# rgal/gym-2048

Hardware: AMD Instinct MI355X
Metric: env-steps/sec at batch=2^20 per MI355X (higher is better)
Workload: dtype u8

## Files before the change

### gym-2048_amd/csrc/g2048_device.h

```cpp
#pragma once

#include <stdint.h>

#if defined(G2048_HOST_CHECK)
#define G2048_DEV static inline
static inline uint32_t g2048_perm(uint32_t hi, uint32_t lo, uint32_t sel)
{
    uint64_t src = ((uint64_t)hi << 32) | lo;
    uint32_t out = 0;
    for (int k = 0; k < 4; ++k) {
        uint32_t s = (sel >> (8 * k)) & 0xff;
        uint32_t byte = s < 8 ? (uint32_t)((src >> (8 * s)) & 0xff) : (s == 12 ? 0u : 0xffu);
        out |= byte << (8 * k);
    }
    return out;
}
static inline uint32_t g2048_mulhi(uint32_t a, uint32_t b) { return (uint32_t)(((uint64_t)a * b) >> 32); }
static inline uint32_t g2048_popc(uint32_t x) { return (uint32_t)__builtin_popcount(x); }
static inline uint32_t g2048_clz(uint32_t x) { return (uint32_t)__builtin_clz(x); }
static inline uint32_t g2048_funnel_shr(uint32_t hi, uint32_t lo, uint32_t k)
{
    return (uint32_t)(((((uint64_t)hi) << 32) | lo) >> (k & 31u));
}
static inline uint32_t g2048_ctz(uint32_t x) { return (uint32_t)__builtin_ctz(x); }
static inline float g2048_rcp(float x) { return 1.0f / x; }
static inline uint32_t g2048_opaque(uint32_t x) { return x; }
static inline uint32_t g2048_bfi(uint32_t m, uint32_t a, uint32_t b) { return (m & a) | (~m & b); }
static inline bool g2048_any(bool x) { return x; }
static inline uint32_t g2048_xor3(uint32_t a, uint32_t b, uint32_t c) { return a ^ b ^ c; }
template <int K> static inline uint32_t g2048_pow2_byte(uint32_t x, uint32_t) { return 1u << ((x >> (8 * K)) & 31u); }
#else
#include <hip/hip_runtime.h>
#define G2048_DEV __device__ __forceinline__
G2048_DEV uint32_t g2048_perm(uint32_t hi, uint32_t lo, uint32_t sel) { return __builtin_amdgcn_perm(hi, lo, sel); }
G2048_DEV uint32_t g2048_mulhi(uint32_t a, uint32_t b) { return __umulhi(a, b); }
G2048_DEV uint32_t g2048_popc(uint32_t x) { return (uint32_t)__popc(x); }
G2048_DEV uint32_t g2048_clz(uint32_t x) { return (uint32_t)__builtin_clz(x); }
G2048_DEV uint32_t g2048_funnel_shr(uint32_t hi, uint32_t lo, uint32_t k) { return __builtin_amdgcn_alignbit(hi, lo, k); }
G2048_DEV uint32_t g2048_ctz(uint32_t x) { return (uint32_t)__builtin_ctz(x); }
G2048_DEV float g2048_rcp(float x) { return __builtin_amdgcn_rcpf(x); }
G2048_DEV uint32_t g2048_opaque(uint32_t x)
{
    asm volatile("" : "+v"(x));
    return x;
}
G2048_DEV uint32_t g2048_bfi(uint32_t m, uint32_t a, uint32_t b) { return __builtin_amdgcn_bitop3_b32(m, a, b, 0xCA); }
G2048_DEV uint32_t g2048_xor3(uint32_t a, uint32_t b, uint32_t c) { return __builtin_amdgcn_bitop3_b32(a, b, c, 0x96); }
template <int K> G2048_DEV uint32_t g2048_pow2_byte(uint32_t x, uint32_t one)
{
    uint32_t r;
    if constexpr (K == 0)
        asm("v_lshlrev_b32_sdwa %0, %1, %2 dst_sel:DWORD dst_unused:UNUSED_PAD src0_sel:BYTE_0 src1_sel:DWORD" : "=v"(r) : "v"(x), "v"(one));
    else if constexpr (K == 1)
        asm("v_lshlrev_b32_sdwa %0, %1, %2 dst_sel:DWORD dst_unused:UNUSED_PAD src0_sel:BYTE_1 src1_sel:DWORD" : "=v"(r) : "v"(x), "v"(one));
    else if constexpr (K == 2)
        asm("v_lshlrev_b32_sdwa %0, %1, %2 dst_sel:DWORD dst_unused:UNUSED_PAD src0_sel:BYTE_2 src1_sel:DWORD" : "=v"(r) : "v"(x), "v"(one));
    else
        asm("v_lshlrev_b32_sdwa %0, %1, %2 dst_sel:DWORD dst_unused:UNUSED_PAD src0_sel:BYTE_3 src1_sel:DWORD" : "=v"(r) : "v"(x), "v"(one));
    return r;
}
G2048_DEV bool g2048_any(bool x) { return __builtin_amdgcn_ballot_w64(x) != 0ull; }
#endif

namespace g2048 {

struct Board {
    uint32_t r[4];
};

#if defined(G2048_HOST_CHECK)
struct uint4 {
    uint32_t x, y, z, w;
};
G2048_DEV Board load_board(const uint4 *boards, uint32_t i)
{
    Board b;
    __builtin_memcpy(b.r, boards + i, 16);
    return b;
}
#else
// ... 151 lines not shown
    bd.r[3] |= tile & h2;
    return n;
}

G2048_DEV uint32_t add_tile(Board &bd, uint32_t w, uint32_t enable = 0xffffffffu)
{
    bool is2;
    return add_tile(bd, w, enable, is2);
}

G2048_DEV bool fresh_is_four_16(uint32_t w1) { return (w1 << 4) > kTwoThreshold; }
G2048_DEV bool fresh_is_four_15(uint32_t w2) { return w2 * 15u > kTwoThreshold; }

G2048_DEV Board fresh_board(uint32_t w1, uint32_t w2)
{
    const uint32_t p1 = w1 >> 28;
    const uint32_t k2 = g2048_mulhi(w2, 15u);
    const uint32_t p2 = k2 + (k2 >= p1 ? 1u : 0u);
    const uint32_t e1 = fresh_is_four_16(w1) ? 2u : 1u;
    const uint32_t e2 = fresh_is_four_15(w2) ? 2u : 1u;
    const uint64_t x1 = (uint64_t)e1 << (8u * (p1 & 7u)), x2 = (uint64_t)e2 << (8u * (p2 & 7u));
    const uint32_t h1 = lanemask_bit0(p1 >> 3), h2 = lanemask_bit0(p2 >> 3);
    const uint32_t x1l = (uint32_t)x1, x1h = (uint32_t)(x1 >> 32), x2l = (uint32_t)x2, x2h = (uint32_t)(x2 >> 32);
    Board bd;
    bd.r[0] = (x1l & ~h1) | (x2l & ~h2);
    bd.r[1] = (x1h & ~h1) | (x2h & ~h2);
    bd.r[2] = (x1l & h1) | (x2l & h2);
    bd.r[3] = (x1h & h1) | (x2h & h2);
    return bd;
}

G2048_DEV bool has_equal_neighbours(const Board &bd)
{
    uint32_t f = 0;
#pragma unroll
    for (int i = 0; i < 4; ++i)
        f |= z80(bd.r[i] ^ (bd.r[i] >> 8)) & 0x00808080u;
#pragma unroll
    for (int i = 0; i < 3; ++i)
        f |= z80(bd.r[i] ^ bd.r[i + 1]);
    return f != 0;
}

G2048_DEV uint32_t max4(uint32_t x, uint32_t y)
{
    const uint32_t ge = mask7(((x | kHigh1) - y) & kHigh1);
    return bfi(ge, x, y);
}

G2048_DEV uint32_t highest(const Board &bd)
{
    uint32_t m = max4(max4(bd.r[0], bd.r[1]), max4(bd.r[2], bd.r[3]));
    m = max4(m, m >> 16);
    m = max4(m, m >> 8);
    return m & 0xffu;
}

G2048_DEV bool is_end(const Board &bd, uint32_t max_exp)
{
    bool end = false;
    if (count_empty(bd) == 0)
        end = !has_equal_neighbours(bd);
    if (max_exp != 0 && highest(bd) == max_exp)
        end = true;
    return end;
}

struct MoveSel {
    uint32_t sa, sb, ta, tc, va, vb;
};

#define G2048_MOVE_LUT_WORDS                                                                        \
    0x03020100u, 0x07060504u, 0x03020100u, 0x07060504u, 0x03020100u, 0x07060504u, 0u, 0u,      \
    0x05010703u, 0x04000602u, 0x05040100u, 0x07060302u, 0x00040206u, 0x01050307u, 0u, 0u,   \
// ... 1123 lines not shown
}

G2048_DEV uint32_t record_deficit(const Board &raw) { return gather12(raw.r[2]) | (gather12(raw.r[3]) << 12); }

G2048_DEV uint32_t record_score(const Board &raw)
{
    return (potential(record_cells(raw)) - record_deficit(raw)) & kScoreMask;
}

G2048_DEV Board make_record(const Board &cells, uint32_t score)
{
    const uint32_t d = (potential(cells) - score) & kScoreMask;
    return Board{{cells.r[0], cells.r[1], cells.r[2] | scatter12(d & 0xfffu), cells.r[3] | scatter12(d >> 12)}};
}

G2048_DEV void record_update(Board &raw, const Board &cells, uint32_t inc_spread)
{
    const uint64_t filled = (static_cast<uint64_t>(raw.r[3] | kCellBits) << 32) | (raw.r[2] | kCellBits);
    const uint64_t sum = filled + inc_spread;
    raw.r[0] = cells.r[0];
    raw.r[1] = cells.r[1];
    raw.r[2] = bfi(kSpareBits, static_cast<uint32_t>(sum), cells.r[2]);
    raw.r[3] = bfi(kSpareBits, static_cast<uint32_t>(sum >> 32), cells.r[3]);
}

G2048_DEV Board fresh_record(uint32_t w1, uint32_t w2)
{
    Board bd = fresh_board(w1, w2);
    const uint32_t fours = (fresh_is_four_16(w1) ? 1u : 0u) + (fresh_is_four_15(w2) ? 1u : 0u);
    bd.r[2] |= fours == 1u ? 0x80u : (fours == 2u ? 0x2000u : 0u);
    return bd;
}

template <class Tables>
G2048_DEV Board fresh_record_lut(uint32_t w1, uint32_t w2, const Tables &tb)
{
    const uint32_t p1 = w1 >> 28;
    const uint32_t k2 = g2048_mulhi(w2, 15u);
    const uint32_t p2 = k2 + (k2 >= p1 ? 1u : 0u);
    const uint32_t s1 = fresh_is_four_16(w1) ? 1u : 0u;
    const uint32_t s2 = fresh_is_four_15(w2) ? 1u : 0u;
    const Board a = tb.onehot_cell(p1), b = tb.onehot_cell(p2);
    const uint32_t fours = s1 + s2;
    Board bd;
    bd.r[0] = (a.r[0] << s1) | (b.r[0] << s2);
    bd.r[1] = (a.r[1] << s1) | (b.r[1] << s2);
    bd.r[2] = (a.r[2] << s1) | (b.r[2] << s2) | ((fours & 1u) << 7) | ((fours >> 1) << 13);
    bd.r[3] = (a.r[3] << s1) | (b.r[3] << s2);
    return bd;
}

G2048_DEV uint32_t onehot_cell_word(uint32_t p, uint32_t j) { return (p >> 2) == j ? 1u << (8u * (p & 3u)) : 0u; }

G2048_DEV uint32_t eq_flags(uint32_t cells, uint32_t splat) { return (kHigh1 - (cells ^ splat)) & kHigh1; }
G2048_DEV uint32_t eq_ones(uint32_t cells, uint32_t splat) { return ((kHigh1 - (cells ^ splat)) >> 7) & 0x01010101u; }

struct OneHot4F16 { uint32_t lo, hi; };
struct OneHot4F32 { uint32_t w[4]; };

G2048_DEV OneHot4F16 onehot4_f16(uint32_t cells, uint32_t splat)
{
    const uint32_t f = eq_flags(cells, splat);
    const uint32_t g = (f - (f >> 7)) & 0x3c3c3c3cu;
    return OneHot4F16{g2048_perm(g, g, 0x010c000cu), g2048_perm(g, g, 0x030c020cu)};
}

G2048_DEV OneHot4F32 onehot4_f32(uint32_t cells, uint32_t splat)
{
    const uint32_t f = eq_flags(cells, splat);
    const uint32_t g = (f - (f >> 7)) & 0x3f3f3f3fu;
    return OneHot4F32{{g2048_perm(g, f, 0x04000c0cu), g2048_perm(g, f, 0x05010c0cu), g2048_perm(g, f, 0x06020c0cu),
                       g2048_perm(g, f, 0x07030c0cu)}};
}

struct alignas(16) Cells16 { uint32_t r[4]; };
struct alignas(16) Chunk16 { uint32_t w[4]; };

template <int OBS>
G2048_DEV Chunk16 onehot_chunk(const Cells16 *recs, uint32_t s, uint32_t lane, uint32_t &board)
{
    if constexpr (OBS == 0) {
// ... 177 lines not shown
```

### gym-2048_amd/csrc/g2048_kernels.hip

```cpp
#include "g2048_kernels.h"

#include "g2048_device.h"
#include "g2048_pcg64.h"

#include <atomic>
#include <type_traits>


namespace g2048 {

constexpr int kBlock = 256;

typedef uint32_t u32x4 __attribute__((ext_vector_type(4)));

__device__ __forceinline__ Board load_board_nt(const uint4 *boards, uint32_t i)
{
    const u32x4 v = __builtin_nontemporal_load(reinterpret_cast<const u32x4 *>(boards) + i);
    return Board{{v.x, v.y, v.z, v.w}};
}

__device__ __forceinline__ void store_board_nt(uint4 *boards, uint32_t i, const Board &b)
{
    const u32x4 v = {b.r[0], b.r[1], b.r[2], b.r[3]};
    __builtin_nontemporal_store(v, reinterpret_cast<u32x4 *>(boards) + i);
}

__device__ __forceinline__ void store_chunk_nt(uint4 *out, uint64_t g, uint32_t a, uint32_t b, uint32_t c, uint32_t d)
{
    const u32x4 v = {a, b, c, d};
    __builtin_nontemporal_store(v, reinterpret_cast<u32x4 *>(out) + g);
}

__device__ __forceinline__ void store_board(uint4 *boards, uint32_t i, const Board &b)
{
    boards[i] = make_uint4(b.r[0], b.r[1], b.r[2], b.r[3]);
}

struct WaveTables {
    uint32_t move[32];
    uint32_t cell[64];
    uint32_t pad[32];
};

#define G2048_CELL_ENTRY(p) ((p) / 4 == 0 ? 1u << (8 * ((p) % 4)) : 0u), ((p) / 4 == 1 ? 1u << (8 * ((p) % 4)) : 0u), \
                            ((p) / 4 == 2 ? 1u << (8 * ((p) % 4)) : 0u), ((p) / 4 == 3 ? 1u << (8 * ((p) % 4)) : 0u)
__device__ const uint32_t kWaveTablesImage[128] __attribute__((aligned(16))) = {
    G2048_MOVE_LUT_WORDS,
    G2048_CELL_ENTRY(0), G2048_CELL_ENTRY(1), G2048_CELL_ENTRY(2), G2048_CELL_ENTRY(3),
    G2048_CELL_ENTRY(4), G2048_CELL_ENTRY(5), G2048_CELL_ENTRY(6), G2048_CELL_ENTRY(7),
    G2048_CELL_ENTRY(8), G2048_CELL_ENTRY(9), G2048_CELL_ENTRY(10), G2048_CELL_ENTRY(11),
    G2048_CELL_ENTRY(12), G2048_CELL_ENTRY(13), G2048_CELL_ENTRY(14), G2048_CELL_ENTRY(15),
};
#undef G2048_CELL_ENTRY

__device__ __forceinline__ uint2 use_after(uint2 x, uint32_t dep)
{
    unsigned long long both = (static_cast<unsigned long long>(x.y) << 32) | x.x;
    asm volatile("" : "+v"(both) : "v"(dep));
    return make_uint2(static_cast<uint32_t>(both), static_cast<uint32_t>(both >> 32));
}

struct LdsTables {
    const WaveTables *t;
    __device__ __forceinline__ MoveSel move_sel(uint32_t action) const
    {
        const uint4 a = *reinterpret_cast<const uint4 *>(t->move + action * 8u);
        const uint2 b = *reinterpret_cast<const uint2 *>(t->move + action * 8u + 4u);
        return MoveSel{a.x, a.y, a.z, a.w, b.x, b.y};
    }
    __device__ __forceinline__ Board onehot_cell(uint32_t p) const
    {
        const uint4 v = *reinterpret_cast<const uint4 *>(t->cell + p * 4u);
        return Board{{v.x, v.y, v.z, v.w}};
    }
};

__device__ __forceinline__ uint2 load_tables_piece()
{
    return reinterpret_cast<const uint2 *>(kWaveTablesImage)[threadIdx.x & 63u];
}

__device__ __forceinline__ LdsTables stage_tables(WaveTables *all, uint2 piece)
{
    reinterpret_cast<uint2 *>(all)[threadIdx.x] = piece;
    __builtin_amdgcn_fence(__ATOMIC_RELEASE, "wavefront");
    __builtin_amdgcn_fence(__ATOMIC_ACQUIRE, "wavefront");
    return LdsTables{all + (threadIdx.x >> 6)};
}

struct Lane { uint32_t i_raw, i; bool valid; };
template <uint32_t BLOCK, bool FULL> __device__ __forceinline__ Lane lane_of(uint32_t n)
{
    const uint32_t i_raw = blockIdx.x * BLOCK + threadIdx.x;
    const bool valid = FULL || i_raw < n;
    return Lane{i_raw, valid ? i_raw : n - 1u, valid};
}

template <int ACT> struct RawAction { typedef uint32_t type; };
template <> struct RawAction<1> { typedef uint8_t type; };
template <> struct RawAction<2> { typedef int32_t type; };
template <> struct RawAction<3> { typedef long long type; };
template <int ACT>
__device__ __forceinline__ typename RawAction<ACT>::type load_action_at(const void *__restrict__ actions, size_t idx)
{
    if constexpr (ACT == 0)
        return 0u;
    else
        return __builtin_nontemporal_load(static_cast<const typename RawAction<ACT>::type *>(actions) + idx);
}

template <class Raw> __device__ __forceinline__ uint32_t action_bits(Raw raw) { return static_cast<uint32_t>(raw) & 3u; }

__device__ __forceinline__ void report_bad_action(unsigned long long *action_err, bool bad, uint32_t raw_low, uint32_t global_index)
{
    const unsigned long long offenders = __builtin_amdgcn_ballot_w64(bad);
    if (offenders == 0ull)
        return;
// ... 1 lines not shown
        __hip_atomic_store(action_err, (1ull << 63) | (static_cast<unsigned long long>(raw_low & 0xffu) << 32) | global_index,
                           __ATOMIC_RELAXED, __HIP_MEMORY_SCOPE_SYSTEM);
}

struct BadAction {
    bool bad = false; uint32_t raw = 0;
    template <class Raw> __device__ __forceinline__ static bool outside(Raw v)
    {
        typedef typename std::make_unsigned<Raw>::type U;
        return static_cast<U>(v) > static_cast<U>(3);
    }
    template <class Raw> __device__ __forceinline__ uint32_t note_only(Raw v)
    {
        const auto w = static_cast<typename std::conditional<(sizeof(Raw) > 4), unsigned long long, uint32_t>::type>(v);
        bad = outside(w);
        raw = static_cast<uint32_t>(w);
        return action_bits(w);
    }
};

__device__ __forceinline__ unsigned long long record_episode_ends(const StepArgs &p, uint32_t i, bool fin, bool illegal,
                                                                  const Board &terminal, uint32_t &episodes, uint32_t &illegal_ends)
{
    const unsigned long long done = __builtin_amdgcn_ballot_w64(fin);
    if (done == 0ull)
        return 0ull;
    if (fin) {
        if (p.st.last_record)
            store_board(p.st.last_record, i, terminal);
        if (p.terminal_boards)
            store_board(p.terminal_boards, i, record_cells(terminal));
    }
    episodes += static_cast<uint32_t>(__popcll(done));
    illegal_ends += static_cast<uint32_t>(__popcll(__builtin_amdgcn_ballot_w64(fin && illegal)));
    return done;
}

__device__ __forceinline__ uint32_t wave_sum_lane63(uint32_t v)
{
    v += static_cast<uint32_t>(__builtin_amdgcn_update_dpp(0, static_cast<int>(v), 0x111, 0xf, 0xf, false));
    v += static_cast<uint32_t>(__builtin_amdgcn_update_dpp(0, static_cast<int>(v), 0x112, 0xf, 0xf, false));
    v += static_cast<uint32_t>(__builtin_amdgcn_update_dpp(0, static_cast<int>(v), 0x114, 0xf, 0xf, false));
    v += static_cast<uint32_t>(__builtin_amdgcn_update_dpp(0, static_cast<int>(v), 0x118, 0xf, 0xf, false));
    v += static_cast<uint32_t>(__builtin_amdgcn_update_dpp(0, static_cast<int>(v), 0x142, 0xa, 0xf, false));
    v += static_cast<uint32_t>(__builtin_amdgcn_update_dpp(0, static_cast<int>(v), 0x143, 0xc, 0xf, false));
    return v;
}

__device__ __forceinline__ unsigned long long wave_sum64_lane63(unsigned long long v)
{
    const uint32_t s0 = wave_sum_lane63(static_cast<uint32_t>(v) & 0x3fffffu);
    const uint32_t s1 = wave_sum_lane63(static_cast<uint32_t>(v >> 22) & 0x3fffffu);
    const uint32_t s2 = wave_sum_lane63(static_cast<uint32_t>(v >> 44));
    return static_cast<unsigned long long>(s0) + (static_cast<unsigned long long>(s1) << 22) +
           (static_cast<unsigned long long>(s2) << 44);
}

struct EpisodeCounters {
    uint32_t *slot;
    uint32_t ep_lo, ill_lo, gain_lo, pend_lo, ep_hi, ill_hi, gain_hi, pend_hi;
};

__device__ __forceinline__ uint32_t *slot_of(unsigned long long *ep_counters, uint32_t wave_id)
{
    return reinterpret_cast<uint32_t *>(ep_counters + kSlotWords * wave_id);
}

__device__ __forceinline__ EpisodeCounters load_episode_counters(const StepArgs &p, uint32_t i_raw)
{
    uint32_t *slot = slot_of(p.st.ep_counters, __builtin_amdgcn_readfirstlane(i_raw >> 6));
    const uint4 lo = *reinterpret_cast<const uint4 *>(slot), hi = *reinterpret_cast<const uint4 *>(slot + 4);
    return EpisodeCounters{slot, lo.x, lo.y, lo.z, lo.w, hi.x, hi.y, hi.z, hi.w};
}

__device__ __forceinline__ unsigned long long slot_get(const uint32_t *slot, uint32_t k)
{
    return static_cast<unsigned long long>(slot[k]) | (static_cast<unsigned long long>(slot[4u + k]) << 32);
}

__device__ __forceinline__ void slot_set(uint32_t *slot, uint32_t k, unsigned long long v)
{
    slot[k] = static_cast<uint32_t>(v);
    slot[4u + k] = static_cast<uint32_t>(v >> 32);
}

enum : uint32_t { kSlotEpisodes = 0, kSlotIllegal = 1, kSlotGain = 2, kSlotPending = 3 };

__device__ __forceinline__ void flush_episode_counts(const EpisodeCounters &c, uint32_t episodes, uint32_t illegal_ends,
                                                     unsigned long long gain_lane63, unsigned long long pending)
{
    if ((threadIdx.x & 63u) != 63u)
        return;
    const unsigned long long ep = (static_cast<unsigned long long>(c.ep_hi) << 32 | c.ep_lo) + episodes;
    const unsigned long long ill = (static_cast<unsigned long long>(c.ill_hi) << 32 | c.ill_lo) + illegal_ends;
    const unsigned long long gain = (static_cast<unsigned long long>(c.gain_hi) << 32 | c.gain_lo) + gain_lane63;
    typedef uint32_t u32x3 __attribute__((ext_vector_type(3)));
    const u32x3 lo = {static_cast<uint32_t>(ep), static_cast<uint32_t>(ill), static_cast<uint32_t>(gain)};
    *reinterpret_cast<u32x3 *>(c.slot) = lo;
    const uint32_t ep_hi = static_cast<uint32_t>(ep >> 32), ill_hi = static_cast<uint32_t>(ill >> 32),
                   gain_hi = static_cast<uint32_t>(gain >> 32);
    if (ep_hi != c.ep_hi || ill_hi != c.ill_hi || gain_hi != c.gain_hi) {
        const u32x3 hi = {ep_hi, ill_hi, gain_hi};
        *reinterpret_cast<u32x3 *>(c.slot + 4) = hi;
    }
    const uint32_t pend_lo = static_cast<uint32_t>(pending), pend_hi = static_cast<uint32_t>(pending >> 32);
    if (pend_lo != c.pend_lo || pend_hi != c.pend_hi) {
        c.slot[3] = pend_lo;
        c.slot[7] = pend_hi;
    }
}

__device__ __forceinline__ unsigned long long pending_after_step(unsigned long long done, uint32_t auto_reset)
{
    return done & (0ull - static_cast<unsigned long long>(auto_reset == 0u ? 1u : 0u));
}

__device__ __forceinline__ void adjust_slot(unsigned long long *ep_counters, uint32_t i_raw, int32_t delta, bool clear)
{
    const uint32_t total = wave_sum_lane63(static_cast<uint32_t>(delta));
    const unsigned long long cleared = __builtin_amdgcn_ballot_w64(clear);
    if ((threadIdx.x & 63u) == 63u) {
        uint32_t *slot = slot_of(ep_counters, i_raw >> 6);
        slot_set(slot, kSlotGain, slot_get(slot, kSlotGain) + static_cast<unsigned long long>(static_cast<long long>(static_cast<int32_t>(total))));
        slot_set(slot, kSlotPending, slot_get(slot, kSlotPending) & ~cleared);
    }
}

__device__ __forceinline__ bool is_pending(unsigned long long *ep_counters, uint32_t i_raw)
{
    const unsigned long long pending = slot_get(slot_of(ep_counters, __builtin_amdgcn_readfirstlane(i_raw >> 6)), kSlotPending);
    return ((pending >> (threadIdx.x & 63u)) & 1ull) != 0ull;
}

constexpr uint32_t kObsOccupancyPad = 58u * 1024u;

static_assert(sizeof(WaveTables) * (kBlock / 64) + sizeof(uint4) * kBlock + kObsOccupancyPad <= 64u * 1024u,
              "static LDS + occupancy pad exceed the 64 KiB workgroup limit");

template <auto Kernel>
static uint32_t obs_pad_for()
{
    static std::atomic<signed char> state[64] = {};
    int dev = 0;
    if (hipGetDevice(&dev) != hipSuccess || dev < 0 || dev >= 64)
        dev = 0;
    signed char known = state[dev].load(std::memory_order_acquire);
    if (known == 0) {
        const hipError_t err = hipFuncSetAttribute(reinterpret_cast<const void *>(Kernel), hipFuncAttributeMaxDynamicSharedMemorySize,
                                                   static_cast<int>(kObsOccupancyPad));
        if (err != hipSuccess)
            (void)hipGetLastError();
        known = err == hipSuccess ? 1 : -1;
        state[dev].store(known, std::memory_order_release);
    }
    return known > 0 ? kObsOccupancyPad : 0u;
}

template <int OBS, bool FULL>
__device__ __forceinline__ void emit_onehot_as(const Cells16 *recs, uint4 *out, uint32_t lane, uint32_t n_here)
{
    constexpr uint32_t kStores = 16u << OBS;
    constexpr uint32_t kUnroll = OBS == 2 ? 16u : kStores;
#pragma unroll kUnroll
    for (uint32_t s = 0; s < kStores; ++s) {
        uint32_t b;
        const Chunk16 c = onehot_chunk<OBS>(recs, s, lane, b);
        if (FULL || b < n_here)
            store_chunk_nt(out, s * 64u + lane, c.w[0], c.w[1], c.w[2], c.w[3]);
    }
}
// ... 80 lines not shown
step_args(uint4 *boards, const void *actions, unsigned long long *ep_counters, uint32_t board_offset, uint32_t seed_lo, uint32_t seed_hi,
          uint32_t t_lo, uint32_t t_hi, uint32_t n, float *reward, const StepTail &tail)
{
    StepArgs p{};
    p.st.boards = boards;
    p.st.last_record = tail.last_record;
    p.st.ep_counters = ep_counters;
    p.actions = actions;
    p.reward = reward;
    p.terminated = tail.terminated;
    p.illegal = STD ? nullptr : tail.illegal;
    p.highest = STD ? nullptr : tail.highest;
    p.terminal_boards = STD ? nullptr : tail.terminal_boards;
    p.n = n;
    p.board_offset = board_offset;
    p.seed_lo = seed_lo;
    p.seed_hi = seed_hi;
    p.t_lo = t_lo;
    p.t_hi = t_hi;
    p.illegal_reward = tail.illegal_reward;
    p.max_exp = STD ? 0u : tail.max_exp;
    p.auto_reset = tail.auto_reset;
    return p;
}

template <int ACT, bool FULL, bool STD, bool HAS_OBS>
__device__ __forceinline__ void step_body(WaveTables *s_tables, uint4 *s_recs, uint4 *boards, const void *actions,
                                          unsigned long long *ep_counters, uint32_t board_offset, uint32_t seed_lo, uint32_t seed_hi,
                                          uint32_t t_lo, uint32_t t_hi, uint32_t n, float *reward, const StepTail &tail)
{
    const StepArgs p = step_args<STD>(boards, actions, ep_counters, board_offset, seed_lo, seed_hi, t_lo, t_hi, n, reward, tail);
    const Lane ln = lane_of<kBlock, FULL>(p.n);
    Board rec = load_board_nt(p.st.boards, ln.i);
    const uint2 tables_piece = load_tables_piece();
    const EpisodeCounters counters = load_episode_counters(p, ln.i_raw);

    const Words w = philox4x32_10(p.t_lo, p.t_hi, p.board_offset + ln.i, 0u, p.seed_lo, p.seed_hi);
    BadAction bad;
    const uint32_t action = ACT == 0 ? w.w[3] >> 30 : bad.note_only(load_action_at<ACT>(p.actions, ln.i));
    const LdsTables tb = stage_tables(s_tables, use_after(tables_piece, w.w[0]));

    const StepOut o = play_record(rec, action, w, p.max_exp, tb);

    uint32_t episodes = 0, illegal_ends = 0;
    const unsigned long long done = record_episode_ends(p, ln.i, o.terminated && ln.valid, !o.legal, rec, episodes, illegal_ends);
    const uint32_t wave_gain = wave_sum_lane63(ln.valid ? o.gain : 0u);
    const unsigned long long pending = pending_after_step(done, p.auto_reset);
    uint32_t top = 0;
    if (p.highest)
        top = highest(record_cells(rec));
    if (o.terminated && p.auto_reset != 0)
        reset_record(rec, o, w, tb);

    if (ln.valid) {
        store_board_nt(p.st.boards, ln.i, rec);
        if (STD || p.reward)
            __builtin_nontemporal_store(o.legal ? static_cast<float>(o.gain) : p.illegal_reward, p.reward + ln.i);
        if (STD || p.terminated)
            __builtin_nontemporal_store(static_cast<uint8_t>(o.terminated ? 1 : 0), p.terminated + ln.i);
        if (p.illegal)
            __builtin_nontemporal_store(static_cast<uint8_t>(o.legal ? 0 : 1), p.illegal + ln.i);
        if (p.highest)
            __builtin_nontemporal_store(static_cast<uint8_t>(top), p.highest + ln.i);
        if (!STD && tail.boards_out)
            store_board(tail.boards_out, ln.i, record_cells(rec));
    }
    flush_episode_counts(counters, episodes, illegal_ends, wave_gain, pending);
    if constexpr (!STD && ACT != 0) {
        if (tail.action_err)
            report_bad_action(tail.action_err, bad.bad && ln.valid, bad.raw, p.board_offset + ln.i);
    }
    if constexpr (HAS_OBS)
        emit_onehot<FULL>(s_recs + (threadIdx.x & ~63u), rec, tail.obs, tail.obs_dtype, ln.i_raw & ~63u, n);
    if (!STD && tail.done_seq)
        signal_done(tail.done_seq, tail.done_value);
}

template <int ACT, bool FULL, bool STD, bool HAS_OBS>
// ... 13 lines not shown
        *t_ptr = value;
}

template <int ACT, bool FULL>
__global__ void __launch_bounds__(kBlock)
step_graph_kernel(uint4 *boards, const void *actions, unsigned long long *ep_counters, uint32_t board_offset, uint32_t seed_lo,
                  uint32_t seed_hi, const unsigned long long *t_ptr, uint32_t n, uint32_t j, float *reward, const StepTail tail)
{
    __shared__ WaveTables s_tables[kBlock / 64];
    const unsigned long long t = *t_ptr + j;
    step_body<ACT, FULL, true, false>(s_tables, nullptr, boards, actions, ep_counters, board_offset, seed_lo, seed_hi,
                                      static_cast<uint32_t>(t), static_cast<uint32_t>(t >> 32), n, reward, tail);
}

constexpr uint32_t kGainFold = 1024;
__global__ void __launch_bounds__(kBlock) rollout_random_kernel(const StepArgs p)
{
    __shared__ WaveTables s_tables[kBlock / 64];
    const Lane ln = lane_of<kBlock, false>(p.n);
    Board rec = load_board(p.st.boards, ln.i);
    const LdsTables tb = stage_tables(s_tables, load_tables_piece());
    const EpisodeCounters counters = load_episode_counters(p, ln.i_raw);
    uint64_t t = (static_cast<uint64_t>(p.t_hi) << 32) | p.t_lo;
    uint32_t episodes = 0, illegal_ends = 0;
    unsigned long long gained = 0;
    for (uint32_t j0 = 0; j0 < p.k_steps; j0 += kGainFold) {
        const uint32_t j1 = p.k_steps - j0 < kGainFold ? p.k_steps : j0 + kGainFold;
        uint32_t gained32 = 0;
        for (uint32_t j = j0; j < j1; ++j, ++t) {
            const Words w = philox4x32_10(static_cast<uint32_t>(t), static_cast<uint32_t>(t >> 32), p.board_offset + ln.i, 0u,
                                          p.seed_lo, p.seed_hi);
            const StepOut o = play_record(rec, w.w[3] >> 30, w, p.max_exp, tb);
            gained32 += o.gain;
            record_episode_ends(p, ln.i, o.terminated && ln.valid, !o.legal, rec, episodes, illegal_ends);
            if (o.terminated)
                reset_record(rec, o, w, tb);
        }
        gained += gained32;
    }
    if (ln.valid)
        store_board(p.st.boards, ln.i, rec);
    flush_episode_counts(counters, episodes, illegal_ends, wave_sum64_lane63(ln.valid ? gained : 0ull), 0ull);
}

constexpr uint32_t kPrefetch = 4;

template <int ACT>
__global__ void __launch_bounds__(kBlock) rollout_fused_kernel(const StepArgs p, uint64_t stride)
{
    __shared__ WaveTables s_tables[kBlock / 64];
    const Lane ln = lane_of<kBlock, false>(p.n);
    const void *__restrict__ actions = p.actions;
    float *__restrict__ reward = p.reward;
    uint8_t *__restrict__ terminated = p.terminated;
    uint8_t *__restrict__ illegal = p.illegal;
    uint8_t *__restrict__ highest_out = p.highest;
    const uint32_t k = p.k_steps;
    typename RawAction<ACT>::type ahead[kPrefetch];
#pragma unroll
    for (uint32_t q = 0; q < kPrefetch; ++q) {
        ahead[q] = load_action_at<ACT>(actions, static_cast<size_t>(q < k ? q : k - 1u) * stride + ln.i);
        asm volatile("" ::: "memory");
    }
    Board rec = load_board_nt(p.st.boards, ln.i);
    const LdsTables tb = stage_tables(s_tables, load_tables_piece());
    const EpisodeCounters counters = load_episode_counters(p, ln.i_raw);
    uint64_t t = (static_cast<uint64_t>(p.t_hi) << 32) | p.t_lo;
    uint32_t episodes = 0, illegal_ends = 0;
    unsigned long long gained = 0;
    uint32_t gained32 = 0;
    unsigned long long ended_last = 0;
    bool bad_action = false;
    uint32_t bad_raw = 0;
    auto one_step = [&](uint32_t j, uint32_t action_in) {
        const size_t o_idx = static_cast<size_t>(j) * stride + ln.i;
        const Words w = philox4x32_10(static_cast<uint32_t>(t), static_cast<uint32_t>(t >> 32), p.board_offset + ln.i, 0u,
                                      p.seed_lo, p.seed_hi);
        ++t;
        const uint32_t action = ACT == 0 ? w.w[3] >> 30 : action_in & 3u;
        const StepOut o = play_record(rec, action, w, p.max_exp, tb);
        gained32 += o.gain;
        ended_last = record_episode_ends(p, ln.i, o.terminated && ln.valid, !o.legal, rec, episodes, illegal_ends);
        if (ln.valid) {
            if (reward)
                __builtin_nontemporal_store(o.legal ? static_cast<float>(o.gain) : p.illegal_reward, reward + o_idx);
            if (terminated)
                __builtin_nontemporal_store(static_cast<uint8_t>(o.terminated ? 1 : 0), terminated + o_idx);
            if (illegal)
                __builtin_nontemporal_store(static_cast<uint8_t>(o.legal ? 0 : 1), illegal + o_idx);
            if (highest_out)
                __builtin_nontemporal_store(static_cast<uint8_t>(highest(record_cells(rec))), highest_out + o_idx);
        }
        if (o.terminated && p.auto_reset != 0)
            reset_record(rec, o, w, tb);
    };
    auto fetch = [&](uint32_t j) { return load_action_at<ACT>(actions, static_cast<size_t>(j < k ? j : k - 1u) * stride + ln.i); };
    auto check = [&](typename RawAction<ACT>::type raw) {
        if constexpr (ACT != 0) {
            if (BadAction::outside(raw)) {
                bad_action = true;
                bad_raw = static_cast<uint32_t>(raw);
            }
        }
        return static_cast<uint32_t>(raw);
    };
    typename RawAction<ACT>::type set_b[kPrefetch];
    uint32_t j0 = 0;
    for (; j0 + 2u * kPrefetch <= k; j0 += 2u * kPrefetch) {
#pragma unroll
        for (uint32_t q = 0; q < kPrefetch; ++q) {
            if constexpr (ACT != 0)
                set_b[q] = fetch(j0 + q + kPrefetch);
            one_step(j0 + q, check(ahead[q]));
        }
#pragma unroll
// ... 468 lines not shown
                       z80((v.w & kCellBits) ^ splat) >> 7);
    } else if constexpr (OBS == 1) {
        const uint64_t board = g >> 5;
        const uint32_t c = static_cast<uint32_t>(g >> 1) & 15u, half = static_cast<uint32_t>(g) & 1u;
        const uint32_t r0 = cells[board * 4 + half * 2] & kCellBits, r1 = cells[board * 4 + half * 2 + 1] & kCellBits;
        uint32_t h[8];
#pragma unroll
        for (int k = 0; k < 4; ++k) {
            h[k] = (((r0 >> (8 * k)) & 0xffu) == c) ? 0x3c00u : 0u;
            h[4 + k] = (((r1 >> (8 * k)) & 0xffu) == c) ? 0x3c00u : 0u;
        }
        store_chunk_nt(out, g, h[0] | (h[1] << 16), h[2] | (h[3] << 16), h[4] | (h[5] << 16), h[6] | (h[7] << 16));
    } else {
        const uint64_t board = g >> 6;
        const uint32_t c = static_cast<uint32_t>(g >> 2) & 15u, row = static_cast<uint32_t>(g) & 3u;
        const uint32_t r = cells[board * 4 + row] & kCellBits;
        uint32_t f[4];
#pragma unroll
        for (int k = 0; k < 4; ++k)
            f[k] = (((r >> (8 * k)) & 0xffu) == c) ? 0x3f800000u : 0u;
        store_chunk_nt(out, g, f[0], f[1], f[2], f[3]);
    }
}

constexpr uint32_t kAfterstateStaticLds = sizeof(WaveTables) * (kBlock / 64) + sizeof(Cells16) * kBlock * 4u;
constexpr uint32_t kAfterstateObsPad = 64u * 1024u - kAfterstateStaticLds;
static_assert(kAfterstateObsPad <= 48u * 1024u, "afterstate occupancy pad needs the dynamic-LDS opt-in");

template <bool PLAIN, bool OBS>
__global__ void __launch_bounds__(kBlock) afterstates_kernel(const uint4 *__restrict__ boards, uint32_t n, const AfterstateOut o)
{
    __shared__ WaveTables s_tables[kBlock / 64];
    __shared__ Cells16 s_after[kBlock * 4];
    const uint2 piece = load_tables_piece();
    const uint32_t i_raw = blockIdx.x * kBlock + threadIdx.x;
    const bool valid = i_raw < n;
    const uint32_t i = valid ? i_raw : n - 1u;
    const Board in = load_board_nt(boards, i);
    const LdsTables tb = stage_tables(s_tables, piece);
    const Board cells = input_cells<PLAIN>(in);
    Board after[4];
    uint32_t gain[4], mask = 0;
#pragma unroll
    for (uint32_t d = 0; d < 4u; ++d) {
        after[d] = cells;
        if (move_sel(after[d], tb.move_sel(d), gain[d]))
            mask |= 1u << d;
    }
    if (valid && o.legal)
        o.legal[i] = static_cast<uint8_t>(mask);
    if (valid && o.score)
        store_chunk_nt(o.score, i, gain[0], gain[1], gain[2], gain[3]);

    const uint32_t lane = threadIdx.x & 63u;
    const uint32_t wave_first = __builtin_amdgcn_readfirstlane(i_raw & ~63u);
    const uint32_t n_after = wave_first < n ? 4u * (n - wave_first < 64u ? n - wave_first : 64u) : 0u;
    Cells16 *recs = s_after + (threadIdx.x & ~63u) * 4u;
#pragma unroll
    for (uint32_t d = 0; d < 4u; ++d) {
        Cells16 &r = recs[lane * 4u + d];
        r.r[0] = after[d].r[0], r.r[1] = after[d].r[1], r.r[2] = after[d].r[2], r.r[3] = after[d].r[3];
    }
    __builtin_amdgcn_fence(__ATOMIC_RELEASE, "wavefront");
    __builtin_amdgcn_fence(__ATOMIC_ACQUIRE, "wavefront");
    if (o.boards) {
#pragma unroll
        for (uint32_t s = 0; s < 4u; ++s) {
// ... 291 lines not shown
__global__ void __launch_bounds__(kBlock) ntuple_stage_kernel(const uint4 *__restrict__ boards, uint32_t n, const NtupleStagedShape sh,
                                                              uint8_t *__restrict__ stage)
{
    const uint32_t i = blockIdx.x * kBlock + threadIdx.x;
    if (i >= n)
        return;
    stage[i] = static_cast<uint8_t>(ntuple_stage(ntuple_stage_mask(ntuple_pack(load_board(boards, i))), sh));
}

template <uint32_t T, class Shape>
__global__ void __launch_bounds__(kBlock) ntuple_play_kernel(const StepArgs p, const Shape sh, uint32_t frac_bits,
                                                             const int32_t *__restrict__ weights, const NtuplePlayOut io)
{
    __shared__ WaveTables s_tables[kBlock / 64];
    const Lane ln = lane_of<kBlock, false>(p.n);
    Board rec = load_board(p.st.boards, ln.i);
    const LdsTables tb = stage_tables(s_tables, load_tables_piece());
    const EpisodeCounters counters = load_episode_counters(p, ln.i_raw);
    uint32_t left = io.games_left ? io.games_left[ln.i] : 1u;
    uint64_t t = (static_cast<uint64_t>(p.t_hi) << 32) | p.t_lo;
    uint32_t episodes = 0, illegal_ends = 0, played = 0, gained32 = 0;
    unsigned long long gained = 0;
    for (uint32_t j = 0; j < p.k_steps; ++j, ++t) {
        const bool go = left != 0u;
        if (__builtin_amdgcn_ballot_w64(go) == 0ull)
            break;
        StepOut o{};
        Words w{};
        if (go)
            o = ntuple_play_step<T>(rec, t, p.board_offset + ln.i, p.seed_lo, p.seed_hi, sh, frac_bits, weights, p.max_exp, tb, w);
        played += go ? 1u : 0u;
        gained32 += o.gain;
        const bool fin = o.terminated && ln.valid;
        record_episode_ends(p, ln.i, fin, !o.legal, rec, episodes, illegal_ends);
        if (o.terminated) {
            if (fin && io.hist)
                atomicAdd(io.hist + highest(record_cells(rec)), 1ull);
            reset_record(rec, o, w, tb);
            if (io.games_left)
                left -= 1u;
        }
        if ((j + 1u) % kGainFold == 0u) {
            gained += gained32;
            gained32 = 0;
        }
    }
    gained += gained32;
    if (ln.valid) {
        store_board(p.st.boards, ln.i, rec);
        if (io.games_left)
            io.games_left[ln.i] = left;
    }
    const unsigned long long pending = ((static_cast<unsigned long long>(counters.pend_hi) << 32) | counters.pend_lo) &
                                       ~__builtin_amdgcn_ballot_w64(played != 0u);
    flush_episode_counts(counters, episodes, illegal_ends, wave_sum64_lane63(ln.valid ? gained : 0ull), pending);
    if (io.moves) {
        const unsigned long long total = wave_sum64_lane63(ln.valid ? played : 0u);
        if ((threadIdx.x & 63u) == 63u && total != 0ull)
            atomicAdd(io.moves, total);
    }
}

template <int ACT>
__global__ void __launch_bounds__(kBlock) play_step_kernel(const StepArgs p, const NtuplePlayOut io)
{
    __shared__ WaveTables s_tables[kBlock / 64];
    const Lane ln = lane_of<kBlock, false>(p.n);
    Board rec = load_board(p.st.boards, ln.i);
    const auto raw = load_action_at<ACT>(p.actions, ln.i);
    const LdsTables tb = stage_tables(s_tables, load_tables_piece());
    const EpisodeCounters counters = load_episode_counters(p, ln.i_raw);
    uint32_t left = io.games_left ? io.games_left[ln.i] : 1u;
    uint32_t episodes = 0, illegal_ends = 0;
    const bool go = left != 0u;
    StepOut o{};
    Words w{};
    BadAction bad;
    if (go) {
        w = philox4x32_10(p.t_lo, p.t_hi, p.board_offset + ln.i, 0u, p.seed_lo, p.seed_hi);
        uint32_t action;
        if constexpr (ACT == 0)
            action = w.w[3] >> 30;
        else
            action = bad.note_only(raw);
        o = play_record(rec, action, w, p.max_exp, tb);
    }
    const bool fin = o.terminated && ln.valid;
    record_episode_ends(p, ln.i, fin, !o.legal, rec, episodes, illegal_ends);
    if (o.terminated) {
        if (fin && io.hist)
            atomicAdd(io.hist + highest(record_cells(rec)), 1ull);
        reset_record(rec, o, w, tb);
        if (io.games_left)
            left -= 1u;
    }
    if (ln.valid) {
        store_board(p.st.boards, ln.i, rec);
        if (io.games_left)
            io.games_left[ln.i] = left;
    }
    const unsigned long long played = __builtin_amdgcn_ballot_w64(go);
    const unsigned long long pending = ((static_cast<unsigned long long>(counters.pend_hi) << 32) | counters.pend_lo) & ~played;
    flush_episode_counts(counters, episodes, illegal_ends, wave_sum_lane63(ln.valid ? o.gain : 0u), pending);
    if (io.moves) {
        const unsigned long long total = static_cast<unsigned long long>(__popcll(played & __builtin_amdgcn_ballot_w64(ln.valid)));
        if ((threadIdx.x & 63u) == 63u && total != 0ull)
            atomicAdd(io.moves, total);
    }
    if constexpr (ACT != 0) {
        if (p.action_err)
            report_bad_action(p.action_err, bad.bad && ln.valid, bad.raw, p.board_offset + ln.i);
    }
}

template <uint32_t T, class Shape>
__global__ void __launch_bounds__(kBlock) ntuple_td_step_kernel(const StepArgs p, const Shape sh, uint32_t frac_bits,
                                                                const int32_t *__restrict__ weights, const NtupleTdIo io)
{
    __shared__ WaveTables s_tables[kBlock / 64];
    const Lane ln = lane_of<kBlock, false>(p.n);
    Board rec = load_board(p.st.boards, ln.i);
// ... 1243 lines not shown
```

Before: 106.9 billion.

## Fold fresh-tile value into LUT, bitop3 neighbour test, reshape counter flush

Result: faster. 108.4 billion, median of 6 (+1.4%).

```diff
diff --git a/gym-2048_amd/csrc/g2048_device.h b/gym-2048_amd/csrc/g2048_device.h
--- a/gym-2048_amd/csrc/g2048_device.h
+++ b/gym-2048_amd/csrc/g2048_device.h
@@ -28,6 +28,9 @@
 static inline uint32_t g2048_bfi(uint32_t m, uint32_t a, uint32_t b) { return (m & a) | (~m & b); }
 static inline bool g2048_any(bool x) { return x; }
 static inline uint32_t g2048_xor3(uint32_t a, uint32_t b, uint32_t c) { return a ^ b ^ c; }
+static inline uint32_t g2048_and3(uint32_t a, uint32_t b, uint32_t c) { return a & b & c; }
+static inline uint32_t g2048_and_or(uint32_t a, uint32_t b, uint32_t c) { return (a & b) | c; }
+static inline uint32_t g2048_xor_and(uint32_t a, uint32_t b, uint32_t c) { return (a ^ b) & c; }
 template <int K> static inline uint32_t g2048_pow2_byte(uint32_t x, uint32_t) { return 1u << ((x >> (8 * K)) & 31u); }
 #else
 #include <hip/hip_runtime.h>
@@ -46,6 +49,9 @@
 }
 G2048_DEV uint32_t g2048_bfi(uint32_t m, uint32_t a, uint32_t b) { return __builtin_amdgcn_bitop3_b32(m, a, b, 0xCA); }
 G2048_DEV uint32_t g2048_xor3(uint32_t a, uint32_t b, uint32_t c) { return __builtin_amdgcn_bitop3_b32(a, b, c, 0x96); }
+G2048_DEV uint32_t g2048_and3(uint32_t a, uint32_t b, uint32_t c) { return __builtin_amdgcn_bitop3_b32(a, b, c, 0x80); }
+G2048_DEV uint32_t g2048_and_or(uint32_t a, uint32_t b, uint32_t c) { return __builtin_amdgcn_bitop3_b32(a, b, c, 0xEA); }
+G2048_DEV uint32_t g2048_xor_and(uint32_t a, uint32_t b, uint32_t c) { return __builtin_amdgcn_bitop3_b32(a, b, c, 0x28); }
 template <int K> G2048_DEV uint32_t g2048_pow2_byte(uint32_t x, uint32_t one)
 {
     uint32_t r;
@@ -263,14 +269,15 @@
 
 G2048_DEV bool has_equal_neighbours(const Board &bd)
 {
-    uint32_t f = 0;
+    uint32_t h[4], v[3];
 #pragma unroll
     for (int i = 0; i < 4; ++i)
-        f |= z80(bd.r[i] ^ (bd.r[i] >> 8)) & 0x00808080u;
+        h[i] = (bd.r[i] ^ (bd.r[i] >> 8)) + kLow7;
 #pragma unroll
     for (int i = 0; i < 3; ++i)
-        f |= z80(bd.r[i] ^ bd.r[i + 1]);
-    return f != 0;
+        v[i] = (bd.r[i] ^ bd.r[i + 1]) + kLow7;
+    const uint32_t rows = g2048_and_or(g2048_and3(h[0], h[1], h[2]), h[3], 0x80000000u);
+    return g2048_and_or(rows, g2048_and3(v[0], v[1], v[2]), kLow7) != 0xffffffffu;
 }
 
 G2048_DEV uint32_t max4(uint32_t x, uint32_t y)
@@ -1460,21 +1467,47 @@
     return bd;
 }
 
+#define G2048_FRESH_TILE_WORD(p, e, j) ((p) / 4 == (j) ? (e) << (8 * ((p) % 4)) : 0u)
+#define G2048_FRESH_TILE_ENTRY(p, e) G2048_FRESH_TILE_WORD(p, e, 0), G2048_FRESH_TILE_WORD(p, e, 1), \
+                                     G2048_FRESH_TILE_WORD(p, e, 2), G2048_FRESH_TILE_WORD(p, e, 3)
+#define G2048_FRESH_TILE_CELL(p) G2048_FRESH_TILE_ENTRY(p, 1u), G2048_FRESH_TILE_ENTRY(p, 2u)
+#define G2048_FRESH_TILE_WORDS                                                                              \
+    G2048_FRESH_TILE_CELL(0), G2048_FRESH_TILE_CELL(1), G2048_FRESH_TILE_CELL(2), G2048_FRESH_TILE_CELL(3),     \
+    G2048_FRESH_TILE_CELL(4), G2048_FRESH_TILE_CELL(5), G2048_FRESH_TILE_CELL(6), G2048_FRESH_TILE_CELL(7),     \
+    G2048_FRESH_TILE_CELL(8), G2048_FRESH_TILE_CELL(9), G2048_FRESH_TILE_CELL(10), G2048_FRESH_TILE_CELL(11),   \
+    G2048_FRESH_TILE_CELL(12), G2048_FRESH_TILE_CELL(13), G2048_FRESH_TILE_CELL(14), G2048_FRESH_TILE_CELL(15)
+
+#if defined(G2048_HOST_CHECK)
+static const uint32_t kFreshTileHost[128] = {G2048_FRESH_TILE_WORDS};
+template <class Tables> G2048_DEV Board fresh_tile(const Tables &, uint32_t e)
+{
+    const uint32_t *v = kFreshTileHost + 4u * e;
+    return Board{{v[0], v[1], v[2], v[3]}};
+}
+#else
+template <class Tables> G2048_DEV Board fresh_tile(const Tables &tb, uint32_t e) { return tb.fresh_tile(e); }
+#endif
+
+G2048_DEV uint32_t fresh_tile_entry(uint32_t p, uint32_t fraction)
+{
+    const uint64_t sum = ((static_cast<uint64_t>(p) << 32) | fraction) + ((static_cast<uint64_t>(p) << 32) | (0xffffffffu - kTwoThreshold));
+    return static_cast<uint32_t>(sum >> 32);
+}
+
 template <class Tables>
 G2048_DEV Board fresh_record_lut(uint32_t w1, uint32_t w2, const Tables &tb)
 {
     const uint32_t p1 = w1 >> 28;
     const uint32_t k2 = g2048_mulhi(w2, 15u);
     const uint32_t p2 = k2 + (k2 >= p1 ? 1u : 0u);
-    const uint32_t s1 = fresh_is_four_16(w1) ? 1u : 0u;
-    const uint32_t s2 = fresh_is_four_15(w2) ? 1u : 0u;
-    const Board a = tb.onehot_cell(p1), b = tb.onehot_cell(p2);
-    const uint32_t fours = s1 + s2;
+    const uint32_t e1 = fresh_tile_entry(p1, w1 << 4), e2 = fresh_tile_entry(p2, w2 * 15u);
+    const Board a = fresh_tile(tb, e1), b = fresh_tile(tb, e2);
+    const uint32_t one_four = g2048_xor_and(e1, e2, 1u), two_fours = g2048_and3(e1, e2, 1u);
     Board bd;
-    bd.r[0] = (a.r[0] << s1) | (b.r[0] << s2);
-    bd.r[1] = (a.r[1] << s1) | (b.r[1] << s2);
-    bd.r[2] = (a.r[2] << s1) | (b.r[2] << s2) | ((fours & 1u) << 7) | ((fours >> 1) << 13);
-    bd.r[3] = (a.r[3] << s1) | (b.r[3] << s2);
+    bd.r[0] = a.r[0] | b.r[0];
+    bd.r[1] = a.r[1] | b.r[1];
+    bd.r[2] = (two_fours << 13) | g2048_opaque((one_four << 7) | (a.r[2] | b.r[2]));
+    bd.r[3] = a.r[3] | b.r[3];
     return bd;
 }
 
diff --git a/gym-2048_amd/csrc/g2048_kernels.hip b/gym-2048_amd/csrc/g2048_kernels.hip
--- a/gym-2048_amd/csrc/g2048_kernels.hip
+++ b/gym-2048_amd/csrc/g2048_kernels.hip
@@ -38,26 +38,21 @@
 
 struct WaveTables {
     uint32_t move[32];
-    uint32_t cell[64];
-    uint32_t pad[32];
+    uint32_t tile[128];
+    uint32_t pad[96];
 };
-
-#define G2048_CELL_ENTRY(p) ((p) / 4 == 0 ? 1u << (8 * ((p) % 4)) : 0u), ((p) / 4 == 1 ? 1u << (8 * ((p) % 4)) : 0u), \
-                            ((p) / 4 == 2 ? 1u << (8 * ((p) % 4)) : 0u), ((p) / 4 == 3 ? 1u << (8 * ((p) % 4)) : 0u)
-__device__ const uint32_t kWaveTablesImage[128] __attribute__((aligned(16))) = {
+static_assert(sizeof(WaveTables) == 64 * sizeof(uint4), "one 16-byte piece per lane");
+
+__device__ const uint32_t kWaveTablesImage[256] __attribute__((aligned(16))) = {
     G2048_MOVE_LUT_WORDS,
-    G2048_CELL_ENTRY(0), G2048_CELL_ENTRY(1), G2048_CELL_ENTRY(2), G2048_CELL_ENTRY(3),
-    G2048_CELL_ENTRY(4), G2048_CELL_ENTRY(5), G2048_CELL_ENTRY(6), G2048_CELL_ENTRY(7),
-    G2048_CELL_ENTRY(8), G2048_CELL_ENTRY(9), G2048_CELL_ENTRY(10), G2048_CELL_ENTRY(11),
-    G2048_CELL_ENTRY(12), G2048_CELL_ENTRY(13), G2048_CELL_ENTRY(14), G2048_CELL_ENTRY(15),
+    G2048_FRESH_TILE_WORDS,
 };
-#undef G2048_CELL_ENTRY
-
-__device__ __forceinline__ uint2 use_after(uint2 x, uint32_t dep)
-{
-    unsigned long long both = (static_cast<unsigned long long>(x.y) << 32) | x.x;
-    asm volatile("" : "+v"(both) : "v"(dep));
-    return make_uint2(static_cast<uint32_t>(both), static_cast<uint32_t>(both >> 32));
+
+__device__ __forceinline__ uint4 use_after(uint4 x, uint32_t dep)
+{
+    u32x4 all = {x.x, x.y, x.z, x.w};
+    asm volatile("" : "+v"(all) : "v"(dep));
+    return make_uint4(all.x, all.y, all.z, all.w);
 }
 
 struct LdsTables {
@@ -68,21 +63,21 @@
         const uint2 b = *reinterpret_cast<const uint2 *>(t->move + action * 8u + 4u);
         return MoveSel{a.x, a.y, a.z, a.w, b.x, b.y};
     }
-    __device__ __forceinline__ Board onehot_cell(uint32_t p) const
+    __device__ __forceinline__ Board fresh_tile(uint32_t e) const
     {
-        const uint4 v = *reinterpret_cast<const uint4 *>(t->cell + p * 4u);
+        const uint4 v = *reinterpret_cast<const uint4 *>(t->tile + e * 4u);
         return Board{{v.x, v.y, v.z, v.w}};
     }
 };
 
-__device__ __forceinline__ uint2 load_tables_piece()
-{
-    return reinterpret_cast<const uint2 *>(kWaveTablesImage)[threadIdx.x & 63u];
-}
-
-__device__ __forceinline__ LdsTables stage_tables(WaveTables *all, uint2 piece)
-{
-    reinterpret_cast<uint2 *>(all)[threadIdx.x] = piece;
+__device__ __forceinline__ uint4 load_tables_piece()
+{
+    return reinterpret_cast<const uint4 *>(kWaveTablesImage)[threadIdx.x & 63u];
+}
+
+__device__ __forceinline__ LdsTables stage_tables(WaveTables *all, uint4 piece)
+{
+    reinterpret_cast<uint4 *>(all)[threadIdx.x] = piece;
     __builtin_amdgcn_fence(__ATOMIC_RELEASE, "wavefront");
     __builtin_amdgcn_fence(__ATOMIC_ACQUIRE, "wavefront");
     return LdsTables{all + (threadIdx.x >> 6)};
@@ -150,7 +145,7 @@
             store_board(p.terminal_boards, i, record_cells(terminal));
     }
     episodes += static_cast<uint32_t>(__popcll(done));
-    illegal_ends += static_cast<uint32_t>(__popcll(__builtin_amdgcn_ballot_w64(fin && illegal)));
+    illegal_ends += static_cast<uint32_t>(__popcll(done & ~__builtin_amdgcn_ballot_w64(!illegal)));
     return done;
 }
 
@@ -162,6 +157,7 @@
     v += static_cast<uint32_t>(__builtin_amdgcn_update_dpp(0, static_cast<int>(v), 0x118, 0xf, 0xf, false));
     v += static_cast<uint32_t>(__builtin_amdgcn_update_dpp(0, static_cast<int>(v), 0x142, 0xa, 0xf, false));
     v += static_cast<uint32_t>(__builtin_amdgcn_update_dpp(0, static_cast<int>(v), 0x143, 0xc, 0xf, false));
+    asm volatile("" : "+v"(v));
     return v;
 }
 
@@ -207,22 +203,25 @@
 __device__ __forceinline__ void flush_episode_counts(const EpisodeCounters &c, uint32_t episodes, uint32_t illegal_ends,
                                                      unsigned long long gain_lane63, unsigned long long pending)
 {
+    const unsigned long long ep = (static_cast<unsigned long long>(c.ep_hi) << 32 | c.ep_lo) + episodes;
+    const unsigned long long ill = (static_cast<unsigned long long>(c.ill_hi) << 32 | c.ill_lo) + illegal_ends;
+    const uint32_t ep_hi = static_cast<uint32_t>(ep >> 32), ill_hi = static_cast<uint32_t>(ill >> 32);
+    const bool counts_carry = ep_hi != c.ep_hi || ill_hi != c.ill_hi;
+    const uint32_t pend_lo = static_cast<uint32_t>(pending), pend_hi = static_cast<uint32_t>(pending >> 32);
+    const bool pend_changed = pend_lo != c.pend_lo || pend_hi != c.pend_hi;
     if ((threadIdx.x & 63u) != 63u)
         return;
-    const unsigned long long ep = (static_cast<unsigned long long>(c.ep_hi) << 32 | c.ep_lo) + episodes;
-    const unsigned long long ill = (static_cast<unsigned long long>(c.ill_hi) << 32 | c.ill_lo) + illegal_ends;
-    const unsigned long long gain = (static_cast<unsigned long long>(c.gain_hi) << 32 | c.gain_lo) + gain_lane63;
+    const uint32_t add_lo = static_cast<uint32_t>(gain_lane63), add_hi = static_cast<uint32_t>(gain_lane63 >> 32);
+    const uint32_t gain_lo = c.gain_lo + add_lo;
+    const uint32_t gain_hi = c.gain_hi + add_hi + (gain_lo < add_lo ? 1u : 0u);
     typedef uint32_t u32x3 __attribute__((ext_vector_type(3)));
-    const u32x3 lo = {static_cast<uint32_t>(ep), static_cast<uint32_t>(ill), static_cast<uint32_t>(gain)};
+    const u32x3 lo = {static_cast<uint32_t>(ep), static_cast<uint32_t>(ill), gain_lo};
     *reinterpret_cast<u32x3 *>(c.slot) = lo;
-    const uint32_t ep_hi = static_cast<uint32_t>(ep >> 32), ill_hi = static_cast<uint32_t>(ill >> 32),
-                   gain_hi = static_cast<uint32_t>(gain >> 32);
-    if (ep_hi != c.ep_hi || ill_hi != c.ill_hi || gain_hi != c.gain_hi) {
+    if (counts_carry || gain_hi != c.gain_hi) {
         const u32x3 hi = {ep_hi, ill_hi, gain_hi};
         *reinterpret_cast<u32x3 *>(c.slot + 4) = hi;
     }
-    const uint32_t pend_lo = static_cast<uint32_t>(pending), pend_hi = static_cast<uint32_t>(pending >> 32);
-    if (pend_lo != c.pend_lo || pend_hi != c.pend_hi) {
+    if (pend_changed) {
         c.slot[3] = pend_lo;
         c.slot[7] = pend_hi;
     }
@@ -250,10 +249,10 @@
     return ((pending >> (threadIdx.x & 63u)) & 1ull) != 0ull;
 }
 
-constexpr uint32_t kObsOccupancyPad = 58u * 1024u;
-
-static_assert(sizeof(WaveTables) * (kBlock / 64) + sizeof(uint4) * kBlock + kObsOccupancyPad <= 64u * 1024u,
-              "static LDS + occupancy pad exceed the 64 KiB workgroup limit");
+constexpr uint32_t kObsOccupancyPad = 56u * 1024u;
+
+static_assert(sizeof(WaveTables) * (kBlock / 64) + sizeof(uint4) * kBlock + kObsOccupancyPad == 64u * 1024u,
+              "static LDS + occupancy pad must be exactly the 64 KiB workgroup limit");
 
 template <auto Kernel>
 static uint32_t obs_pad_for()
@@ -400,7 +399,7 @@
     const StepArgs p = step_args<STD>(boards, actions, ep_counters, board_offset, seed_lo, seed_hi, t_lo, t_hi, n, reward, tail);
     const Lane ln = lane_of<kBlock, FULL>(p.n);
     Board rec = load_board_nt(p.st.boards, ln.i);
-    const uint2 tables_piece = load_tables_piece();
+    const uint4 tables_piece = load_tables_piece();
     const EpisodeCounters counters = load_episode_counters(p, ln.i_raw);
 
     const Words w = philox4x32_10(p.t_lo, p.t_hi, p.board_offset + ln.i, 0u, p.seed_lo, p.seed_hi);
@@ -411,7 +410,7 @@
     const StepOut o = play_record(rec, action, w, p.max_exp, tb);
 
     uint32_t episodes = 0, illegal_ends = 0;
-    const unsigned long long done = record_episode_ends(p, ln.i, o.terminated && ln.valid, !o.legal, rec, episodes, illegal_ends);
+    const unsigned long long done = record_episode_ends(p, ln.i, o.terminated && ln.valid, o.legal_mask == 0u, rec, episodes, illegal_ends);
     const uint32_t wave_gain = wave_sum_lane63(ln.valid ? o.gain : 0u);
     const unsigned long long pending = pending_after_step(done, p.auto_reset);
     uint32_t top = 0;
@@ -491,7 +490,7 @@
                                           p.seed_lo, p.seed_hi);
             const StepOut o = play_record(rec, w.w[3] >> 30, w, p.max_exp, tb);
             gained32 += o.gain;
-            record_episode_ends(p, ln.i, o.terminated && ln.valid, !o.legal, rec, episodes, illegal_ends);
+            record_episode_ends(p, ln.i, o.terminated && ln.valid, o.legal_mask == 0u, rec, episodes, illegal_ends);
             if (o.terminated)
                 reset_record(rec, o, w, tb);
         }
@@ -539,7 +538,7 @@
         const uint32_t action = ACT == 0 ? w.w[3] >> 30 : action_in & 3u;
         const StepOut o = play_record(rec, action, w, p.max_exp, tb);
         gained32 += o.gain;
-        ended_last = record_episode_ends(p, ln.i, o.terminated && ln.valid, !o.legal, rec, episodes, illegal_ends);
+        ended_last = record_episode_ends(p, ln.i, o.terminated && ln.valid, o.legal_mask == 0u, rec, episodes, illegal_ends);
         if (ln.valid) {
             if (reward)
                 __builtin_nontemporal_store(o.legal ? static_cast<float>(o.gain) : p.illegal_reward, reward + o_idx);
@@ -1074,7 +1073,7 @@
 {
     __shared__ WaveTables s_tables[kBlock / 64];
     __shared__ Cells16 s_after[kBlock * 4];
-    const uint2 piece = load_tables_piece();
+    const uint4 piece = load_tables_piece();
     const uint32_t i_raw = blockIdx.x * kBlock + threadIdx.x;
     const bool valid = i_raw < n;
     const uint32_t i = valid ? i_raw : n - 1u;
@@ -1432,7 +1431,7 @@
         played += go ? 1u : 0u;
         gained32 += o.gain;
         const bool fin = o.terminated && ln.valid;
-        record_episode_ends(p, ln.i, fin, !o.legal, rec, episodes, illegal_ends);
+        record_episode_ends(p, ln.i, fin, o.legal_mask == 0u, rec, episodes, illegal_ends);
         if (o.terminated) {
             if (fin && io.hist)
                 atomicAdd(io.hist + highest(record_cells(rec)), 1ull);
@@ -1486,7 +1485,7 @@
         o = play_record(rec, action, w, p.max_exp, tb);
     }
     const bool fin = o.terminated && ln.valid;
-    record_episode_ends(p, ln.i, fin, !o.legal, rec, episodes, illegal_ends);
+    record_episode_ends(p, ln.i, fin, o.legal_mask == 0u, rec, episodes, illegal_ends);
     if (o.terminated) {
         if (fin && io.hist)
             atomicAdd(io.hist + highest(record_cells(rec)), 1ull);
```
